# prannaykaul/lvc

Hardware: AMD Instinct MI355X
Metric: img/s COCO 800x1333 R50-FPN inference (GeneralizedRCNN.forward(batched_inputs) -> Instances, 1000 proposals, 100 detections) (higher is better)
Workload: dtype f32 (conv/GEMM inner products on the fp16 / bf16 matrix cores through fp32-accurate operand splits: two-way fp16 with main + cross fp32 accumulators for the 3x3 and wide 1x1 / FC layers, three-way bf16 for the rest; final boxes/scores closer to the fp64 evaluation than the reference's fp32 CPU path,; 1 GPU; COCO-detection R50-FPN inference, bs=8 synthetic 3x800x1333 per GPU, 1000 pre/post-NMS proposals per level/image, 80 classes, conditioned random-init weights; batch_per_gpu=8, global_batch=8, parallelism=dp1

## Files before the change

### include/lvc_amd.h

```cpp
#ifndef LVC_AMD_H
#define LVC_AMD_H

#ifdef __cplusplus
extern "C" {
#endif

#define LVC_OK 0
#define LVC_ERR_INVALID 1
#define LVC_ERR_HIP 2

int lvc_abi_version(void);
const char* lvc_last_error(void);
void lvc_set_error(const char* fmt, ...);

long long lvc_conv_workspace_bytes(void);
long long lvc_conv_range_words_offset(void);
void lvc_set_range_slot(int slot);
int lvc_range_slot(void);
int lvc_range_slots(void);
int lvc_conv2d_nhwc_f32(const float* x, const float* w_packed, const float* scale, const float* shift,
                        const float* residual, float* y, int N, int H, int W, int C, int K, int R, int S,
                        int stride, int pad, int Kg, int relu, int res_mode, int ldy, int ldr, int mode,
                        void* workspace, void* stream);

// ... 7 lines not shown
                            int res_mode, int ldy, int ldr, void* workspace, void* stream);

int lvc_conv3x3_nhwc_f16x2(const float* x, const unsigned short* w_split, const float* scale, const float* shift,
                           const float* residual, float* y, int N, int H, int W, int C, int K, int Kg, int relu,
                           int res_mode, int ldy, int ldr, void* workspace, void* stream);
int lvc_conv3x3_nhwc_f16s1(const float* x, const unsigned short* w_split, const float* scale, const float* shift,
                           const float* residual, float* y, int N, int H, int W, int C, int K, int Kg, int relu,
                           int res_mode, int ldy, int ldr, void* workspace, void* stream);
int lvc_conv3x3_nhwc_f16x2_pipe(const float* x, const unsigned short* w_split, const float* scale, const float* shift,
                                const float* residual, float* y, int N, int H, int W, int C, int K, int Kg, int relu,
                                int res_mode, int ldy, int ldr, void* workspace, void* stream);
int lvc_conv3x3_nhwc_f16_levels(int oneacc, const float* const* xs, float* const* ys, const int* Hs, const int* Ws, int L,
                                const unsigned short* w_split, const float* scale, const float* shift, int N, int C, int K, int Kg,
                                int relu, void* workspace, void* stream);
int lvc_conv3x3_nhwc_f16_levels_pred(int oneacc, const float* const* xs, float* const* ys, const int* Hs, const int* Ws, int L,
                                     const unsigned short* w_split, const float* scale, const float* shift, int N, int C, int K, int Kg,
                                     int relu, const unsigned short* pred_w, const float* pred_scale, const float* pred_shift, int pred_K,
                                     int pred_rows, int pred_ld, int pred_slot, void* workspace, void* stream);
int lvc_conv3x3_nhwc_f16_layers(int oneacc, const float* const* xs, float* const* ys, const int* Hs, const int* Ws, int L,
                                const unsigned short* const* ws, const float* const* scales, const float* const* shifts, int N, int C,
                                int K, int Kg, int relu, void* workspace, void* stream);
void lvc_set_wino_streamk(int mode);
void lvc_set_nms_reduce_global(int on);
void lvc_set_halo_test_hooks(int ph, int pw, int force);
int lvc_conv3x3_nhwc_wino(const float* x, const unsigned short* u, const float* scale, const float* shift, float* y, int N, int H, int W,
                          int C, int K, int Kpad, int relu, int ldy, void* workspace, void* stream);
int lvc_conv3x3_nhwc_wino_pred(const float* x, const unsigned short* u, const float* scale, const float* shift, float* y, int N, int H,
                               int W, int C, int K, int Kpad, int relu, int ldy, const unsigned short* pred_w, const float* pred_scale,
                               const float* pred_shift, int pred_K, int pred_rows, int pred_slot, void* workspace, void* stream);
int lvc_conv1x1_nhwc_f16x2_pipe(const float* x, const unsigned short* w_split, const float* scale, const float* shift,
                                const float* residual, float* y, int N, int H, int W, int C, int K, int stride, int relu,
                                int res_mode, int ldy, int ldr, void* workspace, void* stream);
int lvc_conv1x1_nhwc_f16s1(const float* x, const unsigned short* w_split, const float* scale, const float* shift,
                           const float* residual, float* y, int N, int H, int W, int C, int K, int stride, int relu,
                           int res_mode, int ldy, int ldr, void* workspace, void* stream);
int lvc_conv3x3_nhwc_f16s1_presplit(const float* x, const unsigned short* w_split, const float* scale, const float* shift, void* y,
                                    int N, int H, int W, int C, int K, int Kg, int next_slot, void* workspace, void* stream);
int lvc_conv1x1_nhwc_f16s1_presplit(const void* x, const unsigned short* w_split, const float* scale, const float* shift,
                                    const float* residual, float* y, int N, int H, int W, int C, int K, int relu,
                                    int res_mode, int ldy, int ldr, void* workspace, void* stream);
int lvc_conv1x1_nhwc_f16s1_w2(const float* x, const unsigned short* w_split, const float* scale, const float* shift,
                              const float* residual, float* y, int N, int H, int W, int C, int K, int Kpad, int stride, int relu,
                              int res_mode, int ldy, int ldr, void* workspace, void* stream);
int lvc_conv1x1_chain_nhwc_f16s1(const float* x, int ldx, const unsigned short* wa, int wa_rows, const float* sa, const float* ta,
                                 const float* residual, int ldr, float* y1, int ldy1, int relu1, const unsigned short* wb,
                                 int wb_rows, const float* sb, const float* tb, float* y2, int ldy2, int relu2, int M, int K1,
// ... 236 lines not shown
```

### lvc_amd/_lib.py

```python
import ctypes
import os

_HERE = os.path.dirname(os.path.abspath(__file__))
_SO = os.environ.get("LVC_AMD_LIB") or os.path.join(_HERE, "liblvc_amd.so")
_lib = None

c_void_p = ctypes.c_void_p
c_int = ctypes.c_int
c_float = ctypes.c_float
c_double = ctypes.c_double
c_longlong = ctypes.c_longlong


class LvcNativeError(RuntimeError):
    pass


def lib():
    global _lib
    if _lib is None:
        if not os.path.exists(_SO):
            raise ImportError(
                "lvc_amd: native library {} not found; build it with "
                "`python -c 'import __graft_entry__ as g; g.build()'` or `make -C lvc_amd/csrc` "
                "(there is no CPU fallback)".format(_SO)
            )
        L = ctypes.CDLL(_SO)
        L.lvc_last_error.restype = ctypes.c_char_p
        L.lvc_batched_nms_workspace_bytes.restype = c_longlong
        L.lvc_tta_merge_workspace_bytes.restype = c_longlong
        L.lvc_group_norm_workspace_bytes.restype = c_longlong
        L.lvc_abi_version.restype = c_int
        L.lvc_set_wino_streamk.restype = None
        if os.environ.get("LVC_WINO_STREAMK", "0") != "0":
            L.lvc_set_wino_streamk(c_int(int(os.environ["LVC_WINO_STREAMK"])))
        L.lvc_set_nms_reduce_global.restype = None
        L.lvc_set_halo_test_hooks.restype = None
        if os.environ.get("LVC_NMS_REDUCE_GLOBAL", "0") != "0":
            L.lvc_set_nms_reduce_global(c_int(1))
        _lib = L
    return _lib


def check(status, what=""):
    if status != 0:
        msg = lib().lvc_last_error().decode("utf-8", "replace")
        lib().lvc_set_range_slot(0)
        raise LvcNativeError("{} failed (status {}): {}".format(what or "lvc_amd native call", status, msg))


def ptr(t):
    if t is None:
        return c_void_p(0)
    return c_void_p(t.data_ptr())


def current_stream(device=None):
    import torch

    return c_void_p(torch.cuda.current_stream(device).cuda_stream)
```

### lvc_amd/csrc/boxes.hip

```cpp
#include "common.h"
#include "select_common.h"
#include <stdlib.h>


extern "C" int lvc_batched_nms(const float*, const float*, const int*, const int*, int, int, double, int,
                               int*, int*, void*, long long, void*);
extern "C" long long lvc_batched_nms_workspace_bytes(int, int);

#define MAXL 8


__device__ __forceinline__ int block_excl_scan_1024(int v, int* sh, int* total) {
  const int lane = threadIdx.x & 63, wave = threadIdx.x >> 6;
  int x = v;
#pragma unroll
  for (int o = 1; o < 64; o <<= 1) {
    int t = __shfl_up(x, o);
    if (lane >= o) x += t;
  }
  __syncthreads();
  if (lane == 63) sh[wave] = x;
  __syncthreads();
  if (threadIdx.x == 0) {
    int s = 0;
    for (int w = 0; w < 16; ++w) { int t = sh[w]; sh[w] = s; s += t; }
    sh[16] = s;
  }
  __syncthreads();
  *total = sh[16];
  return sh[wave] + x - v;
// ... 183 lines not shown
  __shared__ int sh[20];
  const int l = blockIdx.x, b = blockIdx.y, tid = threadIdx.x;
  const int A = lv.A, HW = lv.H[l] * lv.W[l], n = HW * A;
  if (n <= TK_SLICE) return;
  const int k = topk < n ? topk : n;
  const int ld = lv.ld_logit[l];
  const float* lg = lv.logits[l] + (size_t)b * HW * ld;
  const unsigned int* keys = wkeys + (size_t)b * lv.key_off[lv.L] + lv.key_off[l];
  const int* H = hist_all + ((size_t)b * lv.L + l) * TK_HSTRIDE;
  unsigned int T;
  int need_eq;
  topk_prefix(H, 4, k, sh, &T, &need_eq);
  const int n_lt = k - need_eq;
  const int npad = k <= 1024 ? 1024 : TOPK_PAD;
  const u64* ck = ckeys + (size_t)b * Ntot + lv.cand_off[l];
  for (int i = tid; i < npad; i += 1024) sortbuf[i] = i < n_lt ? ck[i] : ~0ull;
  const int tie_total = H[1025];
  __syncthreads();
  if (tie_total <= TOPK_PAD) {
    const int* tl = ties + ((size_t)b * lv.L + l) * TOPK_PAD;
    int tp = 64;
    while (tp < tie_total) tp <<= 1;
    for (int i = tid; i < tp; i += 1024) tiebuf[i] = i < tie_total ? (unsigned int)tl[i] : 0xFFFFFFFFu;
    __syncthreads();
    bitonic_sort_lds(tiebuf, tp);
    for (int r = tid; r < need_eq; r += 1024) sortbuf[n_lt + r] = ((u64)T << 32) | tiebuf[r];
  } else {
    int eq_base = 0;
    for (int i0 = 0; i0 < n && eq_base < need_eq; i0 += 1024) {
      const int i = i0 + tid;
      const bool is_eq = i < n && keys[i] == T;
      int tot;
      const int rank = eq_base + block_excl_scan_1024(is_eq ? 1 : 0, sh, &tot);
      if (is_eq && rank < need_eq) sortbuf[n_lt + rank] = ((u64)T << 32) | (unsigned)i;
      eq_base += tot;
    }
  }
  __syncthreads();
  bitonic_sort_lds(sortbuf, npad);
  for (int r = tid; r < k; r += 1024) {
    const int i = (int)(sortbuf[r] & 0xFFFFFFFFu);
    const int pp = i / A, a = i - pp * A;
    cand_idx[(size_t)b * Ntot + lv.cand_off[l] + r] = i;
    cand_score[(size_t)b * Ntot + lv.cand_off[l] + r] = lg[(size_t)pp * ld + a];
  }
}
// ... 94 lines not shown
        if (sm > s || (sm == s && m < l)) lo = mid + 1; else hi = mid;
      }
      rank += lo;
    }
    if (rank < post_topk) {
      *reinterpret_cast<float4*>(pboxes + ((size_t)b * post_topk + rank) * 4) =
          *reinterpret_cast<const float4*>(sboxes + ((size_t)seg * SN + j) * 4);
      plogits[(size_t)b * post_topk + rank] = s;
    }
  }
  for (int r = nout + tid; r < post_topk; r += 1024) {
    *reinterpret_cast<float4*>(pboxes + ((size_t)b * post_topk + r) * 4) = float4{0.f, 0.f, 0.f, 0.f};
    plogits[(size_t)b * post_topk + r] = 0.f;
  }
  if (tid == 0) out_count[b] = nout;
}


static long long align16(long long x) { return (x + 15) & ~15ll; }

struct RpnPlan {
  int Ntot;
  long long nkeys;
  long long off_keys, off_cscore, off_cidx, off_cboxes, off_cscores2, off_clevels, off_ccount, off_keep, off_hist, off_ckeys, off_ties, off_nms, total;
  long long off_sboxes, off_sscores, off_scount, off_skeep, off_snk, off_snms, snms_bytes;
  int max_slices, SN;
};
static RpnPlan rpn_plan(int B, int L, int A, const int* Hs, const int* Ws, int pre_topk) {
  RpnPlan p;
  p.Ntot = 0; p.nkeys = 0; p.max_slices = 0;
  for (int l = 0; l < L; ++l) {
    long long n = (long long)Hs[l] * Ws[l] * A;
    p.nkeys += n;
    p.Ntot += (int)(n < pre_topk ? n : pre_topk);
    if (n > TK_SLICE) { int sl = (int)((n + TK_SLICE - 1) / TK_SLICE); if (sl > p.max_slices) p.max_slices = sl; }
  }
  long long o = 0;
  p.off_keys = o; o = align16(o + (long long)B * p.nkeys * 4);
  p.off_cscore = o; o = align16(o + (long long)B * p.Ntot * 4);
  p.off_cidx = o; o = align16(o + (long long)B * p.Ntot * 4);
  p.off_cboxes = o; o = align16(o + (long long)B * p.Ntot * 16);
  p.off_cscores2 = o; o = align16(o + (long long)B * p.Ntot * 4);
  p.off_clevels = o; o = align16(o + (long long)B * p.Ntot * 4);
  p.off_ccount = o; o = align16(o + (long long)B * 4);
  p.off_keep = o; o = align16(o + (long long)B * p.Ntot * 4);
  p.off_hist = o; o = align16(o + (long long)B * L * TK_HSTRIDE * 4);
  p.off_ckeys = o; o = align16(o + (long long)B * p.Ntot * 8);
  p.off_ties = o; o = align16(o + (long long)B * L * TOPK_PAD * 4);
  p.off_nms = o; o = align16(o + lvc_batched_nms_workspace_bytes(B, p.Ntot));
  p.SN = 0;
  for (int l = 0; l < L; ++l) {
    long long n = (long long)Hs[l] * Ws[l] * A;
    const int c = (int)(n < pre_topk ? n : pre_topk);
    if (c > p.SN) p.SN = c;
  }
  const long long segs = (long long)B * L;
  p.off_sboxes = o; o = align16(o + segs * p.SN * 16);
  p.off_sscores = o; o = align16(o + segs * p.SN * 4);
  p.off_scount = o; o = align16(o + segs * 4);
  p.off_skeep = o; o = align16(o + segs * p.SN * 4);
  p.off_snk = o; o = align16(o + segs * 4);
  p.snms_bytes = lvc_batched_nms_workspace_bytes((int)segs, p.SN);
  p.off_snms = o; o = align16(o + p.snms_bytes);
  p.total = o;
  return p;
}

extern "C" long long lvc_rpn_proposals_workspace_bytes(int B, int L, int A, const int* Hs, const int* Ws,
                                                       int pre_nms_topk) {
// ... 14 lines not shown
  LVC_CHECK_ARG(post_nms_topk > 0, "post_nms_topk must be positive");
  LVC_CHECK_ARG(logits && deltas && cell_anchors && Hs && Ws && strides && d_image_sizes && out_boxes &&
                    out_logits && d_out_count && workspace, "null pointer");
  RpnPlan p = rpn_plan(B, L, A, Hs, Ws, pre_nms_topk);
  LVC_CHECK_ARG(workspace_bytes >= p.total, "workspace too small");
  RpnLevels lv;
  memset(&lv, 0, sizeof lv);
  lv.L = L; lv.A = A;
  for (int l = 0; l < L; ++l) {
    lv.logits[l] = logits[l]; lv.deltas[l] = deltas[l];
    lv.ld_logit[l] = ld_logit[l]; lv.ld_delta[l] = ld_delta[l];
    lv.H[l] = Hs[l]; lv.W[l] = Ws[l]; lv.stride[l] = strides[l];
    lv.cell_anchors[l] = cell_anchors[l];
    long long n = (long long)Hs[l] * Ws[l] * A;
    lv.key_off[l + 1] = lv.key_off[l] + n;
    lv.cand_off[l + 1] = lv.cand_off[l] + (int)(n < pre_nms_topk ? n : pre_nms_topk);
  }
  char* ws = (char*)workspace;
  hipStream_t st = (hipStream_t)stream;
  unsigned int* keys = (unsigned int*)(ws + p.off_keys);
  float* cand_score = (float*)(ws + p.off_cscore);
  int* cand_idx = (int*)(ws + p.off_cidx);
  const bool multi = p.max_slices > 0;
  if (multi) {
    int* hist = (int*)(ws + p.off_hist);
    u64* ckeys = (u64*)(ws + p.off_ckeys);
    int* ties = (int*)(ws + p.off_ties);
    if (hipMemsetAsync(hist, 0, (size_t)B * L * TK_HSTRIDE * 4, st) != hipSuccess) {
      lvc_set_error("%s: hipMemsetAsync failed", __func__);
      return LVC_ERR_HIP;
    }
    for (int phase = 0; phase <= 4; ++phase)
      hipLaunchKernelGGL(rpn_topk_phase_kernel, dim3(p.max_slices, L, B), dim3(1024), 0, st, lv, pre_nms_topk, keys,
                         hist, ckeys, ties, p.Ntot, phase);
    hipLaunchKernelGGL(rpn_topk_final_kernel, dim3(L, B), dim3(1024), 0, st, lv, pre_nms_topk, keys, hist, ckeys, ties,
                       cand_score, cand_idx, p.Ntot);
  }
  hipLaunchKernelGGL(rpn_topk_kernel, dim3(L, B), dim3(1024), 0, st, lv, pre_nms_topk, keys, cand_score,
                     cand_idx, p.Ntot, multi ? TK_SLICE : 0x7FFFFFFF);
  LVC_CHECK_LAUNCH();
  float* sboxes = (float*)(ws + p.off_sboxes);
  float* sscores = (float*)(ws + p.off_sscores);
  int* scount = (int*)(ws + p.off_scount);
  int* skeep = (int*)(ws + p.off_skeep);
  int* snk = (int*)(ws + p.off_snk);
  hipLaunchKernelGGL(rpn_decode_seg_kernel, dim3(L, B), dim3(1024), 0, st, lv, cand_score, cand_idx, p.Ntot,
                     d_image_sizes, scale_clamp, min_box_size, p.SN, sboxes, sscores, scount);
  LVC_CHECK_LAUNCH();
  const int keep_per_level = post_nms_topk < p.SN ? post_nms_topk : p.SN;
  int rc = lvc_batched_nms(sboxes, sscores, nullptr, scount, B * L, p.SN, nms_thresh, keep_per_level, skeep, snk,
                           ws + p.off_snms, p.snms_bytes, stream);
  if (rc) return rc;
  hipLaunchKernelGGL(rpn_merge_levels_kernel, dim3(B), dim3(1024), 0, st, sboxes, sscores, skeep, snk, L, p.SN,
                     post_nms_topk, out_boxes, out_logits, d_out_count);
  LVC_CHECK_LAUNCH();
  return LVC_OK;
}

__global__ void assign_levels_kernel(const float* __restrict__ boxes, int R, int B, int min_level, int max_level,
                                     float canonical_box_size, float canonical_level, int* __restrict__ levels,
                                     float* __restrict__ rois) {
  const int i = blockIdx.x * blockDim.x + threadIdx.x;
// ... 288 lines not shown
```

### lvc_amd/csrc/nms.hip

```cpp
#include "common.h"

typedef unsigned long long u64;

__device__ __forceinline__ unsigned int ordered_desc_key(float f) {
  if (f == 0.f) f = 0.f;
  unsigned int u = __float_as_uint(f);
  u ^= (u >> 31) ? 0xFFFFFFFFu : 0x80000000u;
  return ~u;
}

template <int NPAD>
__global__ __launch_bounds__(1024) void nms_prep_kernel(const float* __restrict__ boxes,
                                                        const float* __restrict__ scores,
                                                        const int* __restrict__ idxs,
                                                        const int* __restrict__ counts, int Nmax,
                                                        int* __restrict__ order,
                                                        float* __restrict__ sboxes,
                                                        int* __restrict__ sidx) {
  extern __shared__ __attribute__((aligned(16))) unsigned char dsm[];
  u64* keys = reinterpret_cast<u64*>(dsm);
  __shared__ float red[16];
  const int img = blockIdx.x;
  const int tid = threadIdx.x;
  int n = counts ? counts[img] : Nmax;
  if (n > Nmax) n = Nmax;
// ... 35 lines not shown
        int lo = ((t & ~(j - 1)) << 1) | (t & (j - 1));
        int hi = lo | j;
        bool up = (lo & k) == 0;
        u64 a = keys[lo], b = keys[hi];
        if ((a > b) == up) { keys[lo] = b; keys[hi] = a; }
      }
      __syncthreads();
    }
  }
  int* ord = order + (size_t)img * Nmax;
  float* sb = sboxes + (size_t)img * Nmax * 4;
  int* si = sidx + (size_t)img * Nmax;
  for (int r = tid; r < n; r += 1024) {
    int i = (int)(keys[r] & 0xFFFFFFFFu);
    ord[r] = i;
    int id = ix ? ix[i] : 0;
    float off = (float)id * maxp1;
    sb[r * 4 + 0] = bx[i * 4 + 0] + off;
    sb[r * 4 + 1] = bx[i * 4 + 1] + off;
    sb[r * 4 + 2] = bx[i * 4 + 2] + off;
    sb[r * 4 + 3] = bx[i * 4 + 3] + off;
    si[r] = id;
  }
}

#define NMS_MASK_STRIDE 96
#define NMS_TILE 16384
#define NMS_HEAD_MIN 2048
__global__ __launch_bounds__(64) void nms_mask_kernel(const float* __restrict__ sboxes,
                                                      const int* __restrict__ sidx,
                                                      const int* __restrict__ counts, int Nmax,
                                                      int nwords, double thr, u64* __restrict__ mask, int row0,
                                                      int rows_cap, const int* __restrict__ num_keep, int max_keep) {
  const int img = blockIdx.z;
  int n = counts ? counts[img] : Nmax;
  if (n > Nmax) n = Nmax;
  const int nend = n < row0 + rows_cap ? n : row0 + rows_cap;
  if (num_keep && num_keep[img] >= max_keep) return;
  const int nchunks = nend > row0 ? (nend - row0 + 63) >> 6 : 0;
  const int lane = threadIdx.x;
  const float* sb = sboxes + (size_t)img * Nmax * 4;
  const int* si = sidx + (size_t)img * Nmax;
  for (int ci = blockIdx.y; ci < nchunks; ci += gridDim.y) {
  const int i_me = row0 + ci * 64 + lane;
  float ix1 = 0, iy1 = 0, ix2 = 0, iy2 = 0; int iid = -1;
  if (i_me < nend) {
// ... 332 lines not shown
  }
}

static int pad_pow2(int n) {
  int p = 1024;
  while (p < n) p <<= 1;
  return p;
}

static long long pad_pow2_ll(long long n) {
  long long p = NMS_TILE;
  while (p < n) p <<= 1;
  return p;
}

extern "C" long long lvc_batched_nms_workspace_bytes(int B, int Nmax) {
  const long long rows = Nmax < NMS_TILE ? Nmax : NMS_TILE;
  const long long nwords = (rows + 63) / 64;
  long long per = (long long)Nmax * 4 * 4  + (long long)Nmax * 4  +
                  (long long)Nmax * 4  + rows * nwords * 8 ;
  if (Nmax > NMS_TILE)
    per += (long long)Nmax * 4 + NMS_MAX_WORDS * 8 + pad_pow2_ll(Nmax) * 8 + 16;
  else if (Nmax > NMS_HEAD_MIN)
    per += (long long)Nmax * 4 + NMS_MAX_WORDS * 8 + 16;
  return (long long)B * per + 512;
}

static int g_nms_reduce_global = 0;
extern "C" void lvc_set_nms_reduce_global(int on) { g_nms_reduce_global = on; }

extern "C" int lvc_batched_nms(const float* boxes, const float* scores, const int* idxs,
                               const int* d_counts, int B, int Nmax, double iou_threshold,
                               int max_keep, int* keep, int* d_num_keep, void* workspace,
                               long long workspace_bytes, void* stream) {
  LVC_CHECK_ARG(B >= 0 && Nmax >= 0, "negative size");
  if (B == 0) return LVC_OK;
  LVC_CHECK_ARG(d_num_keep, "null d_num_keep");
  hipStream_t st = (hipStream_t)stream;
  if (Nmax == 0) {
    (void)hipMemsetAsync(d_num_keep, 0, sizeof(int) * B, st);
    return LVC_OK;
  }
  LVC_CHECK_ARG(boxes && scores && keep && workspace, "null pointer");
  LVC_CHECK_ARG(workspace_bytes >= lvc_batched_nms_workspace_bytes(B, Nmax), "workspace too small");
  LVC_CHECK_ARG(((uintptr_t)workspace & 15) == 0, "workspace must be 16-byte aligned");
  const int rows_cap = Nmax < NMS_TILE ? Nmax : NMS_TILE;
  const int nwords = (rows_cap + 63) / 64;
  char* ws = (char*)workspace;
  float* sboxes = (float*)ws; ws += (size_t)B * Nmax * 16;
  int* order = (int*)ws; ws += (size_t)B * Nmax * 4;
  int* sidx = (int*)ws; ws += (size_t)B * Nmax * 4;
  ws = (char*)(((uintptr_t)ws + 15) & ~(uintptr_t)15);
  u64* mask = (u64*)ws; ws += (size_t)B * rows_cap * nwords * 8;
  if (max_keep <= 0) max_keep = Nmax;
  const dim3 mask_grid(nwords < NMS_MASK_STRIDE ? nwords : NMS_MASK_STRIDE, nwords, B);

  if (Nmax <= NMS_TILE) {
    const int npad = pad_pow2(Nmax);
    const size_t lds = (size_t)npad * 8;
#define LAUNCH_PREP(NP)                                                                              \
  {                                                                                                  \
    (void)hipFuncSetAttribute((const void*)nms_prep_kernel<NP>, hipFuncAttributeMaxDynamicSharedMemorySize, \
                        (int)lds);                                                                   \
    hipLaunchKernelGGL(nms_prep_kernel<NP>, dim3(B), dim3(1024), lds, st, boxes, scores, idxs,       \
                       d_counts, Nmax, order, sboxes, sidx);                                         \
  }
    switch (npad) {
      case 1024: LAUNCH_PREP(1024); break;
      case 2048: LAUNCH_PREP(2048); break;
      case 4096: LAUNCH_PREP(4096); break;
      case 8192: LAUNCH_PREP(8192); break;
      default: LAUNCH_PREP(16384); break;
    }
#undef LAUNCH_PREP
    LVC_CHECK_LAUNCH();
    int head = ((8 * max_keep + 63) / 64) * 64;
    if (head < 1024) head = 1024;
    if (Nmax > NMS_HEAD_MIN && head * 2 <= Nmax) {
      int* kept_pos = (int*)ws; ws += (size_t)B * Nmax * 4;
      ws = (char*)(((uintptr_t)ws + 15) & ~(uintptr_t)15);
      u64* removed_init = (u64*)ws;
      if (hipMemsetAsync(d_num_keep, 0, sizeof(int) * B, st) != hipSuccess) {
        lvc_set_error("%s: hipMemsetAsync failed", __func__);
        return LVC_ERR_HIP;
      }
      const int hw = head / 64;
      hipLaunchKernelGGL(nms_mask_kernel, dim3(hw < NMS_MASK_STRIDE ? hw : NMS_MASK_STRIDE, hw, B), dim3(64), 0, st, sboxes, sidx,
                         d_counts, Nmax, hw, iou_threshold, mask, 0, head, (const int*)nullptr, max_keep);
      LVC_CHECK_LAUNCH();
      hipLaunchKernelGGL(nms_reduce_kernel, dim3(B), dim3(64), 0, st, mask, order, d_counts, Nmax, hw, max_keep, keep,
                         d_num_keep, 0, head, removed_init, kept_pos, 1);
      LVC_CHECK_LAUNCH();
      const int rest = Nmax - head, rw = (rest + 63) / 64;
      hipLaunchKernelGGL(nms_cross_kernel, dim3(lvc_cdiv(rw, 4), B), dim3(256), 0, st, sboxes, sidx, d_counts, Nmax, rw,
                         iou_threshold, kept_pos, d_num_keep, max_keep, head, rest, removed_init);
      LVC_CHECK_LAUNCH();
      hipLaunchKernelGGL(nms_mask_kernel, dim3(rw < NMS_MASK_STRIDE ? rw : NMS_MASK_STRIDE, rw < 16 ? rw : 16, B), dim3(64), 0, st, sboxes, sidx,
                         d_counts, Nmax, rw, iou_threshold, mask, head, rest, (const int*)d_num_keep, max_keep);
      LVC_CHECK_LAUNCH();
      hipLaunchKernelGGL(nms_reduce_kernel, dim3(B), dim3(64), 0, st, mask, order, d_counts, Nmax, rw, max_keep, keep,
                         d_num_keep, head, rest, removed_init, kept_pos, 1);
      LVC_CHECK_LAUNCH();
      return LVC_OK;
    }
    hipLaunchKernelGGL(nms_mask_kernel, mask_grid, dim3(64), 0, st, sboxes, sidx, d_counts, Nmax, nwords, iou_threshold,
                       mask, 0, rows_cap, (const int*)nullptr, max_keep);
    LVC_CHECK_LAUNCH();
    if (rows_cap <= NMS_LDS_ROWS && !g_nms_reduce_global)
      hipLaunchKernelGGL(nms_reduce_lds_kernel, dim3(B), dim3(256), 0, st, mask, order, d_counts, Nmax, nwords, max_keep, keep, d_num_keep,
                         rows_cap);
    else
      hipLaunchKernelGGL(nms_reduce_kernel, dim3(B), dim3(64), 0, st, mask, order, d_counts, Nmax, nwords, max_keep, keep,
                         d_num_keep, 0, rows_cap, (const u64*)nullptr, (int*)nullptr, 0);
    LVC_CHECK_LAUNCH();
    return LVC_OK;
// ... 48 lines not shown
```

### lvc_amd/csrc/select_common.h

```cpp
#pragma once
#include "common.h"

typedef unsigned long long u64;

__device__ __forceinline__ unsigned int desc_key(float f) {
  if (f == 0.f) f = 0.f;
  unsigned int u = __float_as_uint(f);
  u ^= (u >> 31) ? 0xFFFFFFFFu : 0x80000000u;
  return ~u;
}

template <typename T>
__device__ __forceinline__ void bitonic_sort_lds(T* keys, int npad) {
  for (int k = 2; k <= npad; k <<= 1) {
    for (int j = k >> 1; j > 0; j >>= 1) {
      for (int t = threadIdx.x; t < npad / 2; t += blockDim.x) {
        int lo = ((t & ~(j - 1)) << 1) | (t & (j - 1));
        int hi = lo | j;
        bool up = (lo & k) == 0;
        T a = keys[lo], b = keys[hi];
        if ((a > b) == up) { keys[lo] = b; keys[hi] = a; }
      }
      __syncthreads();
    }
// ... 3 lines not shown
__device__ __forceinline__ void find_digit(const int* __restrict__ h, int krem, int* sh) {
  const int tid = threadIdx.x, lane = tid & 63, wave = tid >> 6;
  int x = 0, incl = 0;
  if (tid < 256) {
    x = h[tid];
    incl = x;
#pragma unroll
    for (int o = 1; o < 64; o <<= 1) {
      const int t = __shfl_up(incl, o);
      if (lane >= o) incl += t;
    }
    if (lane == 63) sh[wave] = incl;
  }
  __syncthreads();
  if (tid < 256) {
    int off = 0;
    for (int w = 0; w < wave; ++w) off += sh[w];
    incl += off;
    if (incl - x < krem && krem <= incl) { sh[8] = tid; sh[9] = incl - x; }
  }
  __syncthreads();
}

__device__ __forceinline__ void apply_deltas(float bx1, float by1, float bx2, float by2, float d0, float d1,
                                             float d2, float d3, float wx, float wy, float ww, float wh,
                                             float scale_clamp, float* o) {
  const float widths = bx2 - bx1, heights = by2 - by1;
  const float ctr_x = bx1 + 0.5f * widths, ctr_y = by1 + 0.5f * heights;
  const float dx = d0 / wx, dy = d1 / wy;
  float dw = d2 / ww, dh = d3 / wh;
  dw = dw > scale_clamp ? scale_clamp : dw;
  dh = dh > scale_clamp ? scale_clamp : dh;
  const float pcx = dx * widths + ctr_x, pcy = dy * heights + ctr_y;
  const float pw = expf(dw) * widths, ph = expf(dh) * heights;
  o[0] = pcx - 0.5f * pw; o[1] = pcy - 0.5f * ph; o[2] = pcx + 0.5f * pw; o[3] = pcy + 0.5f * ph;
}
```

### lvc_amd/kernels.py

```python
import collections
import ctypes

import torch

from . import _lib
from ._lib import LvcNativeError, c_double, c_float, c_int, c_longlong, c_void_p, check, ptr

BK = 32
BN = 128


def _stream(t):
    return c_void_p(torch.cuda.current_stream(t.device).cuda_stream)


def _req_cuda(*ts):
    for t in ts:
        if t is not None and not t.is_cuda:
            raise RuntimeError("lvc_amd kernels need device tensors (got a CPU tensor); there is no CPU path")


class PackedConv:

    __slots__ = ("w", "scale", "shift", "K", "C", "R", "S", "stride", "pad", "Kg", "mode", "_w3", "_w2h", "_w2s", "two_acc",
# ... 1108 lines not shown


def roi_align_fpn_backward_nhwc(grad, shapes, scales, rois, levels, sampling_ratio, aligned, num_valid=None,
                                status=None):
    _req_cuda(grad, rois)
    grad = grad.contiguous().float()
    rois = rois.contiguous().float()
    K, ph, pw, C = grad.shape
    L = len(shapes)
    B = shapes[0][0]
    outs = [torch.empty(*sh, device=grad.device, dtype=torch.float32) for sh in shapes]
    FP = c_void_p * L
    IP = c_int * L
    FL = c_float * L
    if levels is not None:
        assert levels.dtype == torch.int32 and levels.is_contiguous()
    st = _lib.lib().lvc_roi_align_fpn_backward_nhwc(
        ptr(grad), FP(*[o.data_ptr() for o in outs]), IP(*[sh[1] for sh in shapes]), IP(*[sh[2] for sh in shapes]),
        FL(*[float(s) for s in scales]), c_int(L), c_int(B), c_int(C), ptr(rois), ptr(levels), ptr(num_valid),
        c_int(K), c_int(ph), c_int(pw), c_int(sampling_ratio), c_int(1 if aligned else 0), ptr(status),
        _stream(grad))
    check(st, "lvc_roi_align_fpn_backward_nhwc")
    return outs


def batched_nms_batch(boxes, scores, idxs, counts, iou_threshold, max_keep=0):
    _req_cuda(boxes, scores, idxs, counts)
    B, Nmax = scores.shape
    boxes = boxes.contiguous().float()
    scores = scores.contiguous().float()
    if idxs is not None:
        idxs = idxs.contiguous()
        assert idxs.dtype == torch.int32
    keep = torch.empty(B, Nmax, dtype=torch.int32, device=boxes.device)
    num_keep = torch.empty(B, dtype=torch.int32, device=boxes.device)
    wsb = _lib.lib().lvc_batched_nms_workspace_bytes(c_int(B), c_int(Nmax))
    ws = torch.empty(wsb, dtype=torch.uint8, device=boxes.device)
    st = _lib.lib().lvc_batched_nms(
        ptr(boxes), ptr(scores), ptr(idxs), ptr(counts), c_int(B), c_int(Nmax), c_double(iou_threshold),
        c_int(max_keep), ptr(keep), ptr(num_keep), ptr(ws), c_longlong(wsb), _stream(boxes))
    check(st, "lvc_batched_nms")
    return keep, num_keep


def batched_nms(boxes, scores, idxs, iou_threshold):
    n = boxes.shape[0]
# ... 1665 lines not shown
```

Before: 655.1 img/s.

## Use radix-select top-k for RPN proposals and head-only sort in NMS prep

Adds a radix-select path for the RPN pre-NMS top-k. A keys kernel builds a global 12-bit histogram and a single per-level kernel compacts the candidates into LDS, selects the threshold and bitonic-sorts only the top k, replacing the earlier multi-kernel sort. NMS prep gets a matching head kernel that radix-selects and sorts only the head entries; a tail sort kernel runs only if the head NMS did not fill max_keep. Both are on by default (mode 3). The cost is more complex code that relies on large LDS buffers and atomics.

```diff
diff --git a/include/lvc_amd.h b/include/lvc_amd.h
--- a/include/lvc_amd.h
+++ b/include/lvc_amd.h
@@ -53,6 +53,8 @@
                                 int K, int Kg, int relu, void* workspace, void* stream);
 void lvc_set_wino_streamk(int mode);
 void lvc_set_nms_reduce_global(int on);
+void lvc_set_select_onelaunch(int mode);
+int lvc_select_onelaunch(void);
 void lvc_set_halo_test_hooks(int ph, int pw, int force);
 int lvc_conv3x3_nhwc_wino(const float* x, const unsigned short* u, const float* scale, const float* shift, float* y, int N, int H, int W,
                           int C, int K, int Kpad, int relu, int ldy, void* workspace, void* stream);
diff --git a/lvc_amd/_lib.py b/lvc_amd/_lib.py
--- a/lvc_amd/_lib.py
+++ b/lvc_amd/_lib.py
@@ -38,6 +38,9 @@
         L.lvc_set_halo_test_hooks.restype = None
         if os.environ.get("LVC_NMS_REDUCE_GLOBAL", "0") != "0":
             L.lvc_set_nms_reduce_global(c_int(1))
+        L.lvc_set_select_onelaunch.restype = None
+        if os.environ.get("LVC_SELECT_ONELAUNCH", "3") != "3":
+            L.lvc_set_select_onelaunch(c_int(int(os.environ["LVC_SELECT_ONELAUNCH"])))
         _lib = L
     return _lib
 
diff --git a/lvc_amd/csrc/boxes.hip b/lvc_amd/csrc/boxes.hip
--- a/lvc_amd/csrc/boxes.hip
+++ b/lvc_amd/csrc/boxes.hip
@@ -6,6 +6,7 @@
 extern "C" int lvc_batched_nms(const float*, const float*, const int*, const int*, int, int, double, int,
                                int*, int*, void*, long long, void*);
 extern "C" long long lvc_batched_nms_workspace_bytes(int, int);
+extern "C" int lvc_select_onelaunch(void);
 
 #define MAXL 8
 
@@ -235,6 +236,209 @@
     int tp = 64;
     while (tp < tie_total) tp <<= 1;
     for (int i = tid; i < tp; i += 1024) tiebuf[i] = i < tie_total ? (unsigned int)tl[i] : 0xFFFFFFFFu;
+    __syncthreads();
+    bitonic_sort_lds(tiebuf, tp);
+    for (int r = tid; r < need_eq; r += 1024) sortbuf[n_lt + r] = ((u64)T << 32) | tiebuf[r];
+  } else {
+    int eq_base = 0;
+    for (int i0 = 0; i0 < n && eq_base < need_eq; i0 += 1024) {
+      const int i = i0 + tid;
+      const bool is_eq = i < n && keys[i] == T;
+      int tot;
+      const int rank = eq_base + block_excl_scan_1024(is_eq ? 1 : 0, sh, &tot);
+      if (is_eq && rank < need_eq) sortbuf[n_lt + rank] = ((u64)T << 32) | (unsigned)i;
+      eq_base += tot;
+    }
+  }
+  __syncthreads();
+  bitonic_sort_lds(sortbuf, npad);
+  for (int r = tid; r < k; r += 1024) {
+    const int i = (int)(sortbuf[r] & 0xFFFFFFFFu);
+    const int pp = i / A, a = i - pp * A;
+    cand_idx[(size_t)b * Ntot + lv.cand_off[l] + r] = i;
+    cand_score[(size_t)b * Ntot + lv.cand_off[l] + r] = lg[(size_t)pp * ld + a];
+  }
+}
+
+__global__ __launch_bounds__(1024) void rpn_topk_keys_kernel(RpnLevels lv, unsigned int* __restrict__ wkeys,
+                                                             int* __restrict__ ghist) {
+  __shared__ int hist[2 * 4096];
+  const int slice = blockIdx.x, l = blockIdx.y, b = blockIdx.z, tid = threadIdx.x;
+  const int A = lv.A, HW = lv.H[l] * lv.W[l], n = HW * A;
+  const int i0 = slice * TK_SLICE;
+  if (i0 >= n) return;
+  const int ld = lv.ld_logit[l];
+  const float* lg = lv.logits[l] + (size_t)b * HW * ld;
+  unsigned int* keys = wkeys + (size_t)b * lv.key_off[lv.L] + lv.key_off[l];
+  for (int t = tid; t < 2 * 4096; t += 1024) hist[t] = 0;
+  __syncthreads();
+  int* myhist = hist + (tid & 1) * 4096;
+  float v[TK_SLICE / 1024];
+#pragma unroll
+  for (int u = 0; u < TK_SLICE / 1024; ++u) {
+    const int i = i0 + u * 1024 + tid;
+    const int p = i / A, a = i - p * A;
+    v[u] = i < n ? lg[(size_t)p * ld + a] : 0.f;
+  }
+#pragma unroll
+  for (int u = 0; u < TK_SLICE / 1024; ++u) {
+    const int i = i0 + u * 1024 + tid;
+    if (i < n) {
+      const unsigned int key = desc_key(v[u]);
+      keys[i] = key;
+      atomicAdd(&myhist[key >> 20], 1);
+    }
+  }
+  __syncthreads();
+  int* G = ghist + ((size_t)b * lv.L + l) * 4096;
+  for (int t = tid; t < 4096; t += 1024) {
+    const int c = hist[t] + hist[4096 + t];
+    if (c) atomicAdd(&G[t], c);
+  }
+}
+
+#define TK1_CAND 8192
+__global__ __launch_bounds__(1024) void rpn_topk_one_kernel(RpnLevels lv, int topk, unsigned int* __restrict__ wkeys,
+                                                            float* __restrict__ cand_score, int* __restrict__ cand_idx,
+                                                            int Ntot, const int* __restrict__ ghist) {
+  __shared__ u64 sortbuf[TOPK_PAD];
+  __shared__ unsigned int tiebuf[TOPK_PAD];
+  __shared__ int hist[2 * 4096];
+  __shared__ unsigned int ckey[TK1_CAND], cidx[TK1_CAND];
+  __shared__ int sh[20];
+  __shared__ int s_cnt[2];
+  const int l = blockIdx.x, b = blockIdx.y, tid = threadIdx.x;
+  const int A = lv.A, HW = lv.H[l] * lv.W[l], n = HW * A;
+  if (n == 0) return;
+  const int k = topk < n ? topk : n;
+  const int ld = lv.ld_logit[l];
+  const float* lg = lv.logits[l] + (size_t)b * HW * ld;
+  unsigned int* keys = wkeys + (size_t)b * lv.key_off[lv.L] + lv.key_off[l];
+  const int npad = k <= 1024 ? 1024 : TOPK_PAD;
+
+  if (ghist) {
+    const int* G = ghist + ((size_t)b * lv.L + l) * 4096;
+    for (int t = tid; t < 4096; t += 1024) hist[t] = G[t];
+  } else {
+    for (int t = tid; t < 2 * 4096; t += 1024) hist[t] = 0;
+    __syncthreads();
+    int* myhist = hist + (tid & 1) * 4096;
+    for (int i0 = tid; i0 < n; i0 += 8 * 1024) {
+      float v[8];
+#pragma unroll
+      for (int u = 0; u < 8; ++u) {
+        const int i = i0 + u * 1024;
+        const int p = i / A, a = i - p * A;
+        v[u] = i < n ? lg[(size_t)p * ld + a] : 0.f;
+      }
+#pragma unroll
+      for (int u = 0; u < 8; ++u) {
+        const int i = i0 + u * 1024;
+        if (i < n) {
+          const unsigned int key = desc_key(v[u]);
+          keys[i] = key;
+          atomicAdd(&myhist[key >> 20], 1);
+        }
+      }
+    }
+    __syncthreads();
+    for (int t = tid; t < 4096; t += 1024) hist[t] += hist[4096 + t];
+  }
+  find_bin_1024(hist, 4096, k, sh);
+  const unsigned int d0 = (unsigned int)sh[18];
+  const int ncand = sh[19] + hist[d0];
+  if (tid < 2) s_cnt[tid] = 0;
+  __syncthreads();
+  unsigned int T;
+  int need_eq;
+  const unsigned int* skeys = keys;
+  const unsigned int* sidx = nullptr;
+  int m = n;
+  if (ncand <= TK1_CAND) {
+    int a0 = (int)((4 - (((uintptr_t)keys >> 2) & 3)) & 3);
+    if (a0 > n) a0 = n;
+    const int nv = (n - a0) >> 2, tail0 = a0 + 4 * nv;
+    {
+      int i = -1;
+      if (tid < a0) i = tid; else if (tid - a0 < n - tail0) i = tail0 + (tid - a0);
+      if (i >= 0) {
+        const unsigned int key = keys[i];
+        if ((key >> 20) <= d0) {
+          const int slot = atomicAdd(&s_cnt[0], 1);
+          if (slot < TK1_CAND) { ckey[slot] = key; cidx[slot] = (unsigned int)i; }
+        }
+      }
+    }
+    const uint4* kv4 = reinterpret_cast<const uint4*>(keys + a0);
+    for (int v0 = tid; v0 < nv; v0 += 8 * 1024) {
+      uint4 q[8];
+#pragma unroll
+      for (int u = 0; u < 8; ++u) {
+        const int v = v0 + u * 1024;
+        q[u] = uint4{0xFFFFFFFFu, 0xFFFFFFFFu, 0xFFFFFFFFu, 0xFFFFFFFFu};
+        if (v < nv) q[u] = kv4[v];
+      }
+      int cnt = 0;
+#pragma unroll
+      for (int u = 0; u < 8; ++u) {
+        const bool in = v0 + u * 1024 < nv;
+        cnt += (in && (q[u].x >> 20) <= d0) + (in && (q[u].y >> 20) <= d0) + (in && (q[u].z >> 20) <= d0) +
+               (in && (q[u].w >> 20) <= d0);
+      }
+      if (cnt == 0) continue;
+      int slot = atomicAdd(&s_cnt[0], cnt);
+#pragma unroll
+      for (int u = 0; u < 8; ++u) {
+        const int v = v0 + u * 1024;
+        if (v >= nv) continue;
+        const unsigned int kk[4] = {q[u].x, q[u].y, q[u].z, q[u].w};
+#pragma unroll
+        for (int c = 0; c < 4; ++c) {
+          if ((kk[c] >> 20) <= d0) {
+            if (slot < TK1_CAND) { ckey[slot] = kk[c]; cidx[slot] = (unsigned int)(a0 + 4 * v + c); }
+            ++slot;
+          }
+        }
+      }
+    }
+    __syncthreads();
+    m = s_cnt[0] < TK1_CAND ? s_cnt[0] : TK1_CAND;
+    __syncthreads();
+    if (tid == 0) s_cnt[0] = 0;
+    skeys = ckey;
+    sidx = cidx;
+    radix_select_1024(ckey, m, k, false, hist, sh, &T, &need_eq);
+  } else {
+    radix_select_1024(keys, n, k, true, hist, sh, &T, &need_eq);
+  }
+  const int n_lt = k - need_eq;
+
+  for (int i = tid; i < npad; i += 1024) sortbuf[i] = ~0ull;
+  __syncthreads();
+  for (int j0 = tid; j0 < m; j0 += 8 * 1024) {
+    unsigned int kv[8];
+#pragma unroll
+    for (int u = 0; u < 8; ++u) { const int j = j0 + u * 1024; kv[u] = j < m ? skeys[j] : 0xFFFFFFFFu; }
+#pragma unroll
+    for (int u = 0; u < 8; ++u) {
+      const int j = j0 + u * 1024;
+      if (j >= m) continue;
+      const unsigned int i = sidx ? sidx[j] : (unsigned int)j;
+      if (kv[u] < T) {
+        const int slot = atomicAdd(&s_cnt[0], 1);
+        if (slot < TOPK_PAD) sortbuf[slot] = ((u64)kv[u] << 32) | i;
+      } else if (kv[u] == T) {
+        const int slot = atomicAdd(&s_cnt[1], 1);
+        if (slot < TOPK_PAD) tiebuf[slot] = i;
+      }
+    }
+  }
+  __syncthreads();
+  const int tie_total = s_cnt[1];
+  if (tie_total <= TOPK_PAD) {
+    int tp = 64;
+    while (tp < tie_total) tp <<= 1;
+    for (int i = tie_total + tid; i < tp; i += 1024) tiebuf[i] = 0xFFFFFFFFu;
     __syncthreads();
     bitonic_sort_lds(tiebuf, tp);
     for (int r = tid; r < need_eq; r += 1024) sortbuf[n_lt + r] = ((u64)T << 32) | tiebuf[r];
@@ -375,18 +579,19 @@
 struct RpnPlan {
   int Ntot;
   long long nkeys;
-  long long off_keys, off_cscore, off_cidx, off_cboxes, off_cscores2, off_clevels, off_ccount, off_keep, off_hist, off_ckeys, off_ties, off_nms, total;
+  long long off_keys, off_cscore, off_cidx, off_cboxes, off_cscores2, off_clevels, off_ccount, off_keep, off_hist, off_hist12, off_ckeys, off_ties, off_nms, total;
   long long off_sboxes, off_sscores, off_scount, off_skeep, off_snk, off_snms, snms_bytes;
-  int max_slices, SN;
+  int max_slices, all_slices, SN;
 };
 static RpnPlan rpn_plan(int B, int L, int A, const int* Hs, const int* Ws, int pre_topk) {
   RpnPlan p;
-  p.Ntot = 0; p.nkeys = 0; p.max_slices = 0;
+  p.Ntot = 0; p.nkeys = 0; p.max_slices = 0; p.all_slices = 0;
   for (int l = 0; l < L; ++l) {
     long long n = (long long)Hs[l] * Ws[l] * A;
     p.nkeys += n;
     p.Ntot += (int)(n < pre_topk ? n : pre_topk);
     if (n > TK_SLICE) { int sl = (int)((n + TK_SLICE - 1) / TK_SLICE); if (sl > p.max_slices) p.max_slices = sl; }
+    { int sl = (int)((n + TK_SLICE - 1) / TK_SLICE); if (sl > p.all_slices) p.all_slices = sl; }
   }
   long long o = 0;
   p.off_keys = o; o = align16(o + (long long)B * p.nkeys * 4);
@@ -398,6 +603,7 @@
   p.off_ccount = o; o = align16(o + (long long)B * 4);
   p.off_keep = o; o = align16(o + (long long)B * p.Ntot * 4);
   p.off_hist = o; o = align16(o + (long long)B * L * TK_HSTRIDE * 4);
+  p.off_hist12 = o; o = align16(o + (long long)B * L * 4096 * 4);
   p.off_ckeys = o; o = align16(o + (long long)B * p.Ntot * 8);
   p.off_ties = o; o = align16(o + (long long)B * L * TOPK_PAD * 4);
   p.off_nms = o; o = align16(o + lvc_batched_nms_workspace_bytes(B, p.Ntot));
@@ -458,6 +664,21 @@
   float* cand_score = (float*)(ws + p.off_cscore);
   int* cand_idx = (int*)(ws + p.off_cidx);
   const bool multi = p.max_slices > 0;
+  const int sel = lvc_select_onelaunch();
+  if ((sel & 1) && (sel & 4)) {
+    hipLaunchKernelGGL(rpn_topk_one_kernel, dim3(L, B), dim3(1024), 0, st, lv, pre_nms_topk, keys, cand_score, cand_idx,
+                       p.Ntot, (const int*)nullptr);
+  } else if (sel & 1) {
+    int* hist12 = (int*)(ws + p.off_hist12);
+    if (hipMemsetAsync(hist12, 0, (size_t)B * L * 4096 * 4, st) != hipSuccess) {
+      lvc_set_error("%s: hipMemsetAsync failed", __func__);
+      return LVC_ERR_HIP;
+    }
+    if (p.all_slices > 0)
+      hipLaunchKernelGGL(rpn_topk_keys_kernel, dim3(p.all_slices, L, B), dim3(1024), 0, st, lv, keys, hist12);
+    hipLaunchKernelGGL(rpn_topk_one_kernel, dim3(L, B), dim3(1024), 0, st, lv, pre_nms_topk, keys, cand_score, cand_idx,
+                       p.Ntot, (const int*)hist12);
+  } else {
   if (multi) {
     int* hist = (int*)(ws + p.off_hist);
     u64* ckeys = (u64*)(ws + p.off_ckeys);
@@ -474,6 +695,7 @@
   }
   hipLaunchKernelGGL(rpn_topk_kernel, dim3(L, B), dim3(1024), 0, st, lv, pre_nms_topk, keys, cand_score,
                      cand_idx, p.Ntot, multi ? TK_SLICE : 0x7FFFFFFF);
+  }
   LVC_CHECK_LAUNCH();
   float* sboxes = (float*)(ws + p.off_sboxes);
   float* sscores = (float*)(ws + p.off_sscores);
diff --git a/lvc_amd/csrc/nms.hip b/lvc_amd/csrc/nms.hip
--- a/lvc_amd/csrc/nms.hip
+++ b/lvc_amd/csrc/nms.hip
@@ -1,6 +1,5 @@
 #include "common.h"
-
-typedef unsigned long long u64;
+#include "select_common.h"
 
 __device__ __forceinline__ unsigned int ordered_desc_key(float f) {
   if (f == 0.f) f = 0.f;
@@ -82,6 +81,163 @@
     sb[r * 4 + 3] = bx[i * 4 + 3] + off;
     si[r] = id;
   }
+}
+
+#define NMS_HEADSORT_MAX 2048
+__global__ __launch_bounds__(1024) void nms_prep_head_kernel(const float* __restrict__ boxes, const float* __restrict__ scores,
+                                                             const int* __restrict__ idxs, const int* __restrict__ counts,
+                                                             int Nmax, int head, int* __restrict__ order,
+                                                             float* __restrict__ sboxes, int* __restrict__ sidx,
+                                                             float* __restrict__ maxp1_out, int* __restrict__ tail_flag) {
+  __shared__ unsigned int k32[16384];
+  __shared__ u64 hbuf[NMS_HEADSORT_MAX];
+  __shared__ int hist[4096];
+  __shared__ float red[16];
+  __shared__ int sh[20];
+  const int img = blockIdx.x;
+  const int tid = threadIdx.x, lane = tid & 63, wave = tid >> 6;
+  int n = counts ? counts[img] : Nmax;
+  if (n > Nmax) n = Nmax;
+  if (n < 0) n = 0;
+  const float* bx = boxes + (size_t)img * Nmax * 4;
+  const float* sc = scores + (size_t)img * Nmax;
+  const int* ix = idxs ? idxs + (size_t)img * Nmax : nullptr;
+
+  float m = -INFINITY;
+  for (int i = tid; i < n * 4; i += 1024) {
+    float v = bx[i];
+    m = v > m ? v : m;
+  }
+  for (int o = 32; o > 0; o >>= 1) {
+    float t = __shfl_xor(m, o);
+    m = t > m ? t : m;
+  }
+  if (lane == 0) red[wave] = m;
+  __syncthreads();
+  if (tid < 64) {
+    float v = tid < 16 ? red[tid] : -INFINITY;
+    for (int o = 8; o > 0; o >>= 1) {
+      float t = __shfl_xor(v, o);
+      v = t > v ? t : v;
+    }
+    if (tid == 0) red[0] = v;
+  }
+  __syncthreads();
+  const float maxp1 = red[0] + 1.0f;
+  const int h = n < head ? n : head;
+  if (tid == 0) { maxp1_out[img] = maxp1; tail_flag[img] = n > h ? 1 : 0; }
+
+  int* ord = order + (size_t)img * Nmax;
+  float* sb = sboxes + (size_t)img * Nmax * 4;
+  int* si = sidx + (size_t)img * Nmax;
+  for (int i = tid; i < n; i += 1024) k32[i] = ordered_desc_key(sc[i]);
+  __syncthreads();
+  if (n > h) {
+    unsigned int T;
+    int need_eq;
+    radix_select_1024(k32, n, h, false, hist, sh, &T, &need_eq);
+    const int n_lt = h - need_eq;
+    int base_lt = 0, base_eq = 0;
+    for (int i0 = 0; i0 < n; i0 += 1024) {
+      const int i = i0 + tid;
+      const unsigned int key = i < n ? k32[i] : 0xFFFFFFFFu;
+      const bool is_lt = i < n && key < T, is_eq = i < n && key == T;
+      const int v = (is_lt ? 1 : 0) | (is_eq ? 1 << 16 : 0);
+      int x = v;
+#pragma unroll
+      for (int o = 1; o < 64; o <<= 1) {
+        const int t = __shfl_up(x, o);
+        if (lane >= o) x += t;
+      }
+      __syncthreads();
+      if (lane == 63) sh[wave] = x;
+      __syncthreads();
+      int excl = x - v, tot = 0;
+      for (int w = 0; w < 16; ++w) { const int t = sh[w]; if (w < wave) excl += t; tot += t; }
+      const int lt_before = base_lt + (excl & 0xFFFF), eq_before = base_eq + (excl >> 16);
+      if (is_lt) {
+        hbuf[lt_before] = ((u64)key << 32) | (unsigned)i;
+      } else if (is_eq && eq_before < need_eq) {
+        hbuf[n_lt + eq_before] = ((u64)key << 32) | (unsigned)i;
+      } else if (i < n) {
+        const int r = h + i - lt_before - (eq_before < need_eq ? eq_before : need_eq);
+        ord[r] = i;
+        const int id = ix ? ix[i] : 0;
+        const float off = (float)id * maxp1;
+        sb[r * 4 + 0] = bx[i * 4 + 0] + off;
+        sb[r * 4 + 1] = bx[i * 4 + 1] + off;
+        sb[r * 4 + 2] = bx[i * 4 + 2] + off;
+        sb[r * 4 + 3] = bx[i * 4 + 3] + off;
+        si[r] = id;
+      }
+      base_lt += tot & 0xFFFF;
+      base_eq += tot >> 16;
+    }
+  } else {
+    for (int i = tid; i < n; i += 1024) hbuf[i] = ((u64)k32[i] << 32) | (unsigned)i;
+  }
+  const int npad = h <= 1024 ? 1024 : NMS_HEADSORT_MAX;
+  for (int i = h + tid; i < npad; i += 1024) hbuf[i] = ~0ull;
+  __syncthreads();
+  bitonic_sort_lds(hbuf, npad);
+  for (int r = tid; r < h; r += 1024) {
+    const int i = (int)(hbuf[r] & 0xFFFFFFFFu);
+    ord[r] = i;
+    const int id = ix ? ix[i] : 0;
+    const float off = (float)id * maxp1;
+    sb[r * 4 + 0] = bx[i * 4 + 0] + off;
+    sb[r * 4 + 1] = bx[i * 4 + 1] + off;
+    sb[r * 4 + 2] = bx[i * 4 + 2] + off;
+    sb[r * 4 + 3] = bx[i * 4 + 3] + off;
+    si[r] = id;
+  }
+}
+
+__global__ __launch_bounds__(1024) void nms_tail_sort_kernel(const float* __restrict__ boxes, const float* __restrict__ scores,
+                                                             const int* __restrict__ idxs, const int* __restrict__ counts,
+                                                             int Nmax, int head, int max_keep,
+                                                             const int* __restrict__ num_keep,
+                                                             const float* __restrict__ maxp1_in, int* __restrict__ tail_flag,
+                                                             int* __restrict__ order, float* __restrict__ sboxes,
+                                                             int* __restrict__ sidx) {
+  extern __shared__ __attribute__((aligned(16))) unsigned char dsm[];
+  u64* keys = reinterpret_cast<u64*>(dsm);
+  const int img = blockIdx.x, tid = threadIdx.x;
+  if (num_keep[img] >= max_keep || !tail_flag[img]) return;
+  int n = counts ? counts[img] : Nmax;
+  if (n > Nmax) n = Nmax;
+  const int mt = n - head;
+  const float* bx = boxes + (size_t)img * Nmax * 4;
+  const float* sc = scores + (size_t)img * Nmax;
+  const int* ix = idxs ? idxs + (size_t)img * Nmax : nullptr;
+  int* ord = order + (size_t)img * Nmax + head;
+  float* sb = sboxes + ((size_t)img * Nmax + head) * 4;
+  int* si = sidx + (size_t)img * Nmax + head;
+  const float maxp1 = maxp1_in[img];
+  int npad = 1024;
+  while (npad < mt) npad <<= 1;
+  for (int r = tid; r < npad; r += 1024) {
+    u64 key = ~0ull;
+    if (r < mt) {
+      const int i = ord[r];
+      key = ((u64)ordered_desc_key(sc[i]) << 32) | (unsigned)i;
+    }
+    keys[r] = key;
+  }
+  __syncthreads();
+  bitonic_sort_lds(keys, npad);
+  for (int r = tid; r < mt; r += 1024) {
+    const int i = (int)(keys[r] & 0xFFFFFFFFu);
+    ord[r] = i;
+    const int id = ix ? ix[i] : 0;
+    const float off = (float)id * maxp1;
+    sb[r * 4 + 0] = bx[i * 4 + 0] + off;
+    sb[r * 4 + 1] = bx[i * 4 + 1] + off;
+    sb[r * 4 + 2] = bx[i * 4 + 2] + off;
+    sb[r * 4 + 3] = bx[i * 4 + 3] + off;
+    si[r] = id;
+  }
+  if (tid == 0) tail_flag[img] = 0;
 }
 
 #define NMS_MASK_STRIDE 96
@@ -460,12 +616,15 @@
   if (Nmax > NMS_TILE)
     per += (long long)Nmax * 4 + NMS_MAX_WORDS * 8 + pad_pow2_ll(Nmax) * 8 + 16;
   else if (Nmax > NMS_HEAD_MIN)
-    per += (long long)Nmax * 4 + NMS_MAX_WORDS * 8 + 16;
+    per += (long long)Nmax * 4 + NMS_MAX_WORDS * 8 + 16 + 16 ;
   return (long long)B * per + 512;
 }
 
 static int g_nms_reduce_global = 0;
 extern "C" void lvc_set_nms_reduce_global(int on) { g_nms_reduce_global = on; }
+static int g_select_onelaunch = 3;
+extern "C" void lvc_set_select_onelaunch(int mode) { g_select_onelaunch = mode; }
+extern "C" int lvc_select_onelaunch(void) { return g_select_onelaunch; }
 
 extern "C" int lvc_batched_nms(const float* boxes, const float* scores, const int* idxs,
                                const int* d_counts, int B, int Nmax, double iou_threshold,
@@ -494,6 +653,10 @@
   const dim3 mask_grid(nwords < NMS_MASK_STRIDE ? nwords : NMS_MASK_STRIDE, nwords, B);
 
   if (Nmax <= NMS_TILE) {
+    int head = ((8 * max_keep + 63) / 64) * 64;
+    if (head < 1024) head = 1024;
+    const bool head_form = Nmax > NMS_HEAD_MIN && head * 2 <= Nmax;
+    const bool head_sort = head_form && head <= NMS_HEADSORT_MAX && (g_select_onelaunch & 2);
     const int npad = pad_pow2(Nmax);
     const size_t lds = (size_t)npad * 8;
 #define LAUNCH_PREP(NP)                                                                              \
@@ -503,7 +666,7 @@
     hipLaunchKernelGGL(nms_prep_kernel<NP>, dim3(B), dim3(1024), lds, st, boxes, scores, idxs,       \
                        d_counts, Nmax, order, sboxes, sidx);                                         \
   }
-    switch (npad) {
+    if (!head_sort) switch (npad) {
       case 1024: LAUNCH_PREP(1024); break;
       case 2048: LAUNCH_PREP(2048); break;
       case 4096: LAUNCH_PREP(4096); break;
@@ -512,12 +675,17 @@
     }
 #undef LAUNCH_PREP
     LVC_CHECK_LAUNCH();
-    int head = ((8 * max_keep + 63) / 64) * 64;
-    if (head < 1024) head = 1024;
-    if (Nmax > NMS_HEAD_MIN && head * 2 <= Nmax) {
+    if (head_form) {
       int* kept_pos = (int*)ws; ws += (size_t)B * Nmax * 4;
       ws = (char*)(((uintptr_t)ws + 15) & ~(uintptr_t)15);
-      u64* removed_init = (u64*)ws;
+      u64* removed_init = (u64*)ws; ws += (size_t)B * NMS_MAX_WORDS * 8;
+      float* maxp1 = (float*)ws; ws += (size_t)B * 4;
+      int* tail_flag = (int*)ws;
+      if (head_sort) {
+        hipLaunchKernelGGL(nms_prep_head_kernel, dim3(B), dim3(1024), 0, st, boxes, scores, idxs, d_counts, Nmax, head, order,
+                           sboxes, sidx, maxp1, tail_flag);
+        LVC_CHECK_LAUNCH();
+      }
       if (hipMemsetAsync(d_num_keep, 0, sizeof(int) * B, st) != hipSuccess) {
         lvc_set_error("%s: hipMemsetAsync failed", __func__);
         return LVC_ERR_HIP;
@@ -529,6 +697,12 @@
       hipLaunchKernelGGL(nms_reduce_kernel, dim3(B), dim3(64), 0, st, mask, order, d_counts, Nmax, hw, max_keep, keep,
                          d_num_keep, 0, head, removed_init, kept_pos, 1);
       LVC_CHECK_LAUNCH();
+      if (head_sort) {
+        (void)hipFuncSetAttribute((const void*)nms_tail_sort_kernel, hipFuncAttributeMaxDynamicSharedMemorySize, (int)lds);
+        hipLaunchKernelGGL(nms_tail_sort_kernel, dim3(B), dim3(1024), lds, st, boxes, scores, idxs, d_counts, Nmax, head,
+                           max_keep, (const int*)d_num_keep, (const float*)maxp1, tail_flag, order, sboxes, sidx);
+        LVC_CHECK_LAUNCH();
+      }
       const int rest = Nmax - head, rw = (rest + 63) / 64;
       hipLaunchKernelGGL(nms_cross_kernel, dim3(lvc_cdiv(rw, 4), B), dim3(256), 0, st, sboxes, sidx, d_counts, Nmax, rw,
                          iou_threshold, kept_pos, d_num_keep, max_keep, head, rest, removed_init);
diff --git a/lvc_amd/csrc/select_common.h b/lvc_amd/csrc/select_common.h
--- a/lvc_amd/csrc/select_common.h
+++ b/lvc_amd/csrc/select_common.h
@@ -49,6 +49,66 @@
   __syncthreads();
 }
 
+__device__ __forceinline__ void find_bin_1024(const int* __restrict__ h, int nbins, int krem, int* sh) {
+  const int tid = threadIdx.x, lane = tid & 63, wave = tid >> 6;
+  __syncthreads();
+  int c[4] = {0, 0, 0, 0};
+  if (tid * 4 < nbins) {
+#pragma unroll
+    for (int u = 0; u < 4; ++u) c[u] = h[tid * 4 + u];
+  }
+  const int s = c[0] + c[1] + c[2] + c[3];
+  int incl = s;
+#pragma unroll
+  for (int o = 1; o < 64; o <<= 1) {
+    const int t = __shfl_up(incl, o);
+    if (lane >= o) incl += t;
+  }
+  if (lane == 63) sh[wave] = incl;
+  __syncthreads();
+  int excl = incl - s;
+  for (int w = 0; w < wave; ++w) excl += sh[w];
+  if (excl < krem && krem <= excl + s) {
+    int u = 0;
+    while (excl + c[u] < krem) { excl += c[u]; ++u; }
+    sh[18] = tid * 4 + u;
+    sh[19] = excl;
+  }
+  __syncthreads();
+}
+
+__device__ __forceinline__ void radix_select_1024(const unsigned int* keys, int n, int k, bool first, int* hist, int* sh,
+                                                  unsigned int* T, int* need_eq) {
+  const int tid = threadIdx.x;
+  unsigned int prefix = 0, pmask = 0;
+  int krem = k;
+  for (int pass = 0; pass < 3; ++pass) {
+    const int shift = pass == 0 ? 20 : pass == 1 ? 8 : 0, nb = pass == 2 ? 256 : 4096;
+    if (pass > 0 || !first) {
+      __syncthreads();
+      for (int t = tid; t < nb; t += 1024) hist[t] = 0;
+      __syncthreads();
+      for (int i0 = tid; i0 < n; i0 += 8 * 1024) {
+        unsigned int kv[8];
+#pragma unroll
+        for (int u = 0; u < 8; ++u) { const int i = i0 + u * 1024; kv[u] = i < n ? keys[i] : 0u; }
+#pragma unroll
+        for (int u = 0; u < 8; ++u) {
+          const int i = i0 + u * 1024;
+          if (i < n && (kv[u] & pmask) == prefix) atomicAdd(&hist[(kv[u] >> shift) & (nb - 1)], 1);
+        }
+      }
+    }
+    find_bin_1024(hist, nb, krem, sh);
+    prefix |= (unsigned int)sh[18] << shift;
+    pmask |= (unsigned int)(nb - 1) << shift;
+    krem -= sh[19];
+  }
+  __syncthreads();
+  *T = prefix;
+  *need_eq = krem;
+}
+
 __device__ __forceinline__ void apply_deltas(float bx1, float by1, float bx2, float by2, float d0, float d1,
                                              float d2, float d3, float wx, float wy, float ww, float wh,
                                              float scale_clamp, float* o) {
diff --git a/lvc_amd/kernels.py b/lvc_amd/kernels.py
--- a/lvc_amd/kernels.py
+++ b/lvc_amd/kernels.py
@@ -1154,6 +1154,15 @@
         _stream(grad))
     check(st, "lvc_roi_align_fpn_backward_nhwc")
     return outs
+
+
+SELECT_ONELAUNCH = int(_os.environ.get("LVC_SELECT_ONELAUNCH", "3"))
+
+
+def set_select_onelaunch(mode):
+    global SELECT_ONELAUNCH
+    SELECT_ONELAUNCH = int(mode)
+    _lib.lib().lvc_set_select_onelaunch(c_int(int(mode)))
 
 
 def batched_nms_batch(boxes, scores, idxs, counts, iou_threshold, max_keep=0):
```

After: 662.7 img/s (median of 6 runs). 1.01x the previous value.
